# Brown-LEMS/Edge_Based_Visual_Odometry

Hardware: AMD Instinct MI355X
Metric: stereo pairs/sec (TOED+NCC match) on KITTI 1241×376; achieved HBM GB/s (higher is better)
Workload: dtype f64; 1 GPU; configs[1]: single KITTI-shaped stereo pair 1241x376 (generator S2, scene 7+rank, 12 px disparity), TOED both images (fp64, no FMA, bit-exact) + epipolar/disparity/orientation candidate search + NCC, resident in HBM, replayed; toed_mode=hybrid, edges_left=126184, edges_right=126340, candidate_pairs=581657, ncc_matches=472947, sims_stored=False, pairs_in_flight_per_gpu=6, streams_per_gpu=4, pairs_submitted_as_hipgraph=2331, toed_strict_fallbacks=0, parallelism=1 independent sequence(s), one per GPU, no collective

## Files before the change

edge_based_visual_odometry_amd/csrc/ebvo_capi.hip:

```cpp
#include <chrono>
#include <cmath>
#include <cstdio>
#include <cstdlib>
#include <cstring>
#include <new>
#include <utility>

#include "ebvo_internal.h"

const char *const g_kernel_names[K_NUM] = {
    "toed_conv",   "toed_nms",   "toed_rowscan", "toed_compact", "toed_finalize", "toed_exact_centre", "toed_exact_mags", "cand_boxes", "epi_lines",
    "cand_count",  "scan",       "cand_fill",    "edge_patches", "ncc_pairs",     "ncc_stored", "misc", "sobel", "gn_refine", "sift",
    "gt_misc",     "gt_pool",    "gt_census",    "gt_rows",      "tgt_project",   "tgt_veridical", "tgt_rows",
    "pose_cascade"};

int ebvo_fail_hip(ebvo_ctx *ctx, hipError_t e, const char *what, const char *file, int line)
{
    char buf[512];
    snprintf(buf, sizeof buf, "%s failed: %s (%s:%d)", what, hipGetErrorString(e), file, line);
    if (ctx)
        ctx->last_error = buf;
    else
        fprintf(stderr, "[ebvo] %s\n", buf);
    (void)hipGetLastError();
// ... 5090 lines not shown
        EBVO_HIP(ctx, hipMemcpyAsync(base + o_pr, proj_right, sizeof(double) * 2 * nz, hipMemcpyHostToDevice, st));
        if (row_on)
            EBVO_HIP(ctx, hipMemcpyAsync(base + o_on, row_on, nz, hipMemcpyHostToDevice, st));
        else
            EBVO_HIP(ctx, hipMemsetAsync(base + o_on, 1, nz, st));
        EBVO_HIP(ctx, hipMemsetAsync(d_rows, 0, sizeof(int32_t) * 2 * nz, st));
    }
    if ((rc = tgt_rows_enqueue(ctx, s, (const int32_t *)(base + o_rp), (const ebvo_edge *)base, (const ebvo_edge *)(base + o_R), nullptr,
                               nullptr, nullptr, nullptr, (const double *)(base + o_pl), (const double *)(base + o_pr),
                               (const uint8_t *)(base + o_on), n_kf, np, tp_dist, d_rows, (uint8_t *)(base + o_tp), d_tot)))
        return rc;
    std::vector<int32_t> rows(2 * nz + 1);
    unsigned long long tot[5] = {0, 0, 0, 0, 0};
    if (n_kf)
        EBVO_HIP(ctx, hipMemcpyAsync(rows.data(), d_rows, sizeof(int32_t) * 2 * nz, hipMemcpyDeviceToHost, st));
    if (is_tp && np)
        EBVO_HIP(ctx, hipMemcpyAsync(is_tp, base + o_tp, npz, hipMemcpyDeviceToHost, st));
    EBVO_HIP(ctx, hipMemcpyAsync(tot, d_tot, sizeof tot, hipMemcpyDeviceToHost, st));
    EBVO_HIP(ctx, hipStreamSynchronize(st));
    tgt_stage_doubles(rows.data(), row_on, n_kf, stage_out);
    if ((rc = tgt_totals_agree(ctx, *stage_out, tot)))
        return rc;
    if (n_tp && n_kf)
        memcpy(n_tp, rows.data(), sizeof(int32_t) * 2 * nz);
    return EBVO_OK;
}

static bool debug_value_ok(int key, int value)
{
    switch (key)
    {
    case 4: case 7: case 10: case 13: case 14:
        return value <= 1;
    case 8:
        return value == 2 || value == 3;
    case 6:
        return value >= 1;
    case 11: case 12:
        return value <= EBVO_DEBUG_MAX_EXACT_BLOCKS;
    case 9:
        return value <= EBVO_DEBUG_MAX_GN_BLOCKS;
    case 18:
        return value <= 512;
    case 19:
        return value <= EBVO_TOTAL_PARTS;
    case 20:
        return value <= 1 << 20;
    case 21:
        return value <= EBVO_DEBUG_MAX_GT_BLOCKS;
    case 22:
        return value <= EBVO_DEBUG_MAX_TEMPORAL_BLOCKS;
    case EBVO_DEBUG_KEY_FINALIZE_BLOCKS:
        return value <= EBVO_DEBUG_MAX_FINALIZE_BLOCKS;
    case 0: case 1: case 2: case 3: case 5: case 15: case 16: case 17:
        return true;
    default:
        return false;
    }
}

extern "C" int ebvo_debug_set(ebvo_ctx *ctx, int key, int value)
{
    if (!ctx || value < 0 || !debug_value_ok(key, value))
        return EBVO_ERR_ARG;
    ++ctx->graph_gen;
    if (key == 10)
        ctx->use_graphs = value;
    else if (key == 14)
        ctx->no_prep = value;
    else if (key == 11 || key == 12)
        ctx->exact_blocks[key - 11] = value;
    else if (key == 15)
        ctx->repeat_mask = value;
    else if (key == 16)
        ctx->stop_stage = value;
    else if (key == 17)
        ctx->ncc_blocks = value;
    else if (key == 18)
        ctx->small_div = value;
    else if (key == 19)
        ctx->cand_blocks = value;
    else if (key == 20)
        ctx->pose_batch = value;
    else if (key == 21)
        ctx->gt_blocks = value;
    else if (key == 22)
        ctx->temporal_blocks = value;
    else if (key == EBVO_DEBUG_KEY_FINALIZE_BLOCKS)
        ctx->finalize_blocks = value;
    else if (key == 13)
        ctx->ingest_stream = value;
    else if (key == 0)
        ctx->wait_attempts = value;
    else if (key == 1)
        ctx->force_overflow = value;
    else if (key == 2)
        ctx->lanes = value;
    else if (key == 3)
        ctx->prof_only = value - 1;
    else if (key == 4)
        ctx->gn_no_rows = value;
    else if (key == 5)
        ctx->gn_rows_below = value;
    else if (key == 9)
        ctx->gn_persist_blocks = value;
    else if (key == 8)
        ctx->gn_persist_waves = value;
    else if (key == 7)
        ctx->gn_per_iteration_rows = value;
    else
    {
        for (Slot *sl : ctx->slots)
            if (sl->tq_cap > 0 && !sl->tq_in_flight)
                sl->tq_cap = value;
    }
    return EBVO_OK;
}

extern "C" int ebvo_fp64_peak(ebvo_ctx *ctx, int iters, double *tflops_muladd, double *tflops_fma)
{
    if (!ctx || iters <= 0)
        return EBVO_ERR_ARG;
    EBVO_HIP(ctx, hipSetDevice(ctx->device));
    return misc_fp64_peak(ctx, *ctx->slots[0], iters, tflops_muladd, tflops_fma);
}
```

edge_based_visual_odometry_amd/csrc/ebvo_internal.h:

```cpp
#ifndef EBVO_INTERNAL_H
#define EBVO_INTERNAL_H

#include <hip/hip_runtime.h>

#include <cstddef>
#include <cstdint>
#include <string>
#include <vector>

#include "../../include/ebvo_hip.h"

enum KernelId
{
    K_CONV = 0,
    K_NMS,
    K_ROWSCAN,
    K_COMPACT,
    K_FINALIZE,
    K_EXACT_CENTRE,
    K_EXACT_MAGS,
    K_BOXES,
    K_LINES,
    K_CAND_COUNT,
    K_SCAN,
// ... 235 lines not shown
    std::vector<Slot *> slots;
    int kf_n = -1;
    uint64_t kf_gen = 0;
    ebvo_edge *kf_L = nullptr, *kf_R = nullptr;
    float *kf_Ln = nullptr, *kf_Rn = nullptr;
    uint8_t *kf_Lf = nullptr, *kf_Rf = nullptr;
    uint8_t *kf_Ld = nullptr, *kf_Rd = nullptr;
    uint8_t *kf_imgL = nullptr, *kf_imgR = nullptr;
    size_t kf_img_bytes = 0;
    int kf_h = 0, kf_w = 0;
    size_t kf_cap = 0;
    bool undist_on = false;
    ebvo_undistort_params undist{};
    int lanes = 4;
    int prof_only = -1;
    uint64_t submit_seq = 0;
    std::vector<hipStream_t> lane_streams;
    hipStream_t copy_stream = nullptr;
    struct HostRange
    {
        const uint8_t *host = nullptr, *dev = nullptr;
        size_t bytes = 0;
        bool ours = false;
    };
    std::vector<HostRange> host_ranges;
    int64_t pull_uploads = 0, stream_uploads = 0;
    hipStream_t upload_stream = nullptr;
    uint64_t sw_seq = 0;
    uint64_t sw_tag[2] = {0, 0};
    int sw_h = 0, sw_w = 0;
    PinnedBuf sw_toed[2], sw_cand, sw_ncc, sw_up;
    int gn_no_rows = 0;
    int gn_persist_waves = 2;
    int gn_persist_blocks = 0;
    int gn_per_iteration_rows = 0;
    int gn_rows_below = 0;
    int wait_attempts = 0;
    int force_overflow = 0;
    uint64_t graph_gen = 1;
    int use_graphs = 1;
    int64_t graph_launches = 0;
    int exact_blocks[2] = {0, 0};
    int cand_blocks = 0;
    int small_div = 0;
    int ncc_blocks = 0;
    int stop_stage = 0;
    int repeat_mask = 0;
    int no_prep = 0;
    int ingest_stream = 0;
    PoseRng pose_rng;
    int pose_batch = 0;
    int gt_blocks = 0;
    int temporal_blocks = 0;
    int finalize_blocks = 0;
    bool screen_audit = false;
    int64_t toed_fallbacks = 0;

    bool prof = false;
    int prof_every = 1;
    int64_t prof_submits = 0;
    std::vector<ProfEvent> prof_free;
    double prof_ms[K_NUM] = {0};
    int64_t prof_launches[K_NUM] = {0};
};

int ebvo_fail_hip(ebvo_ctx *ctx, hipError_t e, const char *what, const char *file, int line);

struct DevCount
{
    int64_t host;
    const int32_t *dev;
};
#ifdef __HIPCC__
__device__ inline int64_t devcount(const DevCount &c)
{
    if (!c.dev)
        return c.host;
    const int64_t v = *c.dev;
    return v < c.host ? v : c.host;
}
#endif

#define EBVO_HIP(ctx, call)                                              \
    do                                                                   \
    {                                                                    \
        hipError_t e_ = (call);                                          \
        if (e_ != hipSuccess)                                            \
            return ebvo_fail_hip((ctx), e_, #call, __FILE__, __LINE__);  \
    } while (0)

int ebvo_grow(ebvo_ctx *ctx, Slot &s, GrowBuf &b, size_t bytes);

bool ebvo_prof_begin(ebvo_ctx *ctx, Slot &s, int kid);
void ebvo_prof_end(ebvo_ctx *ctx, Slot &s);

bool ebvo_prof_kernel(ebvo_ctx *ctx, Slot &s, int kid, hipEvent_t *a, hipEvent_t *b);

struct ProfScope
{
    ebvo_ctx *c;
    Slot &s;
    bool on;
    ProfScope(ebvo_ctx *ctx, Slot &slot, int kid) : c(ctx), s(slot), on(ebvo_prof_begin(ctx, slot, kid)) {}
    ~ProfScope()
    {
        if (on)
// ... 192 lines not shown
```

edge_based_visual_odometry_amd/csrc/toed_kernels.hip:

```cpp
#include <cstring>

#include <hip/hip_ext.h>

#include "ebvo_internal.h"
#include <atomic>
#include "ebvo_math.h"

namespace
{

const double h_TAP_INT[4][19] = {
    {7.99187055345274e-06, 6.69151128824427e-05, 0.000436341347522880, 0.00221592420596900,
     0.00876415024678427, 0.0269954832565940, 0.0647587978329459, 0.120985362259572, 0.176032663382150,
     0.199471140200716, 0.176032663382150, 0.120985362259572, 0.0647587978329459, 0.0269954832565940,
     0.00876415024678427, 0.00221592420596900, 0.000436341347522880, 6.69151128824427e-05,
     7.99187055345274e-06},
    {1.79817087452687e-05, 0.000133830225764885, 0.000763597358165040, 0.00332388630895351,
     0.0109551878084803, 0.0269954832565940, 0.0485690983747094, 0.0604926811297858, 0.0440081658455374, 0,
     -0.0440081658455374, -0.0604926811297858, -0.0485690983747094, -0.0269954832565940,
     -0.0109551878084803, -0.00332388630895351, -0.000763597358165040, -0.000133830225764885,
     -1.79817087452687e-05},
    {3.84608770384913e-05, 0.000250931673309160, 0.00122721003990810, 0.00443184841193801,
     0.0115029471989044, 0.0202466124424455, 0.0202371243227956, 0, -0.0330061243841531,
     -0.0498677850501791, -0.0330061243841531, 0, 0.0202371243227956, 0.0202466124424455,
// ... 1003 lines not shown
                f[7] += cc[3] * rr[0];
                f[8] += cc[0] * rr[3];
            }
            else
            {
                EBVO_ACCUM9(f, cc, rr)
            }
        }
    }
}

template <int SY, int SX>
__device__ inline double exact_mag(const uint8_t *__restrict__ img, int h, int w, const ExactTaps &L, int I, int J)
{
    constexpr bool IP = (SY == 0 && SX == 0);
    const int i = I >> 1, j = J >> 1;
    const double(*ck)[4] = L.tap[SX];
    const double(*rk)[4] = L.tap[SY];
    double fx = 0.0, fy = 0.0;
    constexpr int PM = IP ? 8 : 9;
    const bool fast = __all(window_inside(h, w, i, j));
    const ColMask cm = column_mask(w, j);
    Row24 nxt = fetch_row(img, h, w, i + PM, j);
#pragma unroll 1
    for (int p = -PM; p <= PM; ++p)
    {
        const Row24 cur = nxt;
        nxt = fetch_row(img, h, w, i - min(p + 1, PM), j);
        int vb[19];
        unpack_row(cur, h, i - p, cm, fast, vb);
        const double r0 = rk[p + 9][0], r1 = rk[p + 9][1];
        int lz = 0;
        asm volatile("" : "+v"(lz));
        const double(*ckl)[4] = ck + lz;
#pragma unroll
        for (int q = -PM; q <= PM; ++q)
        {
            const double v = (double)vb[q + 9];
            if (IP)
            {
                fx += v * L.prod[p + 8][q + 8][0];
                fy += v * L.prod[p + 8][q + 8][1];
            }
            else
            {
                fx += (v * ckl[q + 9][1]) * r0;
                fy += (v * ckl[q + 9][0]) * r1;
            }
        }
    }
    return sqrt(fx * fx + fy * fy);
}

#ifdef EBVO_WAVE_TRACE
__device__ unsigned long long g_wave_trace[2][8192 * 4];
__device__ inline void wave_trace(int which, int wave, unsigned long long t0, int tasks)
{
    if ((threadIdx.x & 63) == 0 && wave < 8192)
    {
        const unsigned hw = __builtin_amdgcn_s_getreg(4 | (0 << 6) | (31 << 11));
        const unsigned xcc = __builtin_amdgcn_s_getreg(20 | (0 << 6) | (31 << 11));
        unsigned long long *o = g_wave_trace[which] + (size_t)wave * 4;
        o[0] = t0;
        o[1] = __builtin_amdgcn_s_memrealtime();
        o[2] = ((unsigned long long)xcc << 32) | hw;
        o[3] = (unsigned long long)tasks;
    }
}
extern "C" int ebvo_wave_trace_read(int which, unsigned long long *dst, int n_waves)
{
    return (int)hipMemcpyFromSymbol(dst, HIP_SYMBOL(g_wave_trace), (size_t)n_waves * 32, (size_t)which * 8192 * 32,
                                    hipMemcpyDeviceToHost);
}
#define EBVO_TRACE_BEGIN() const unsigned long long trace_t0 = __builtin_amdgcn_s_memrealtime(); int trace_n = 0
#define EBVO_TRACE_TASK() ++trace_n
#define EBVO_TRACE_END(which) wave_trace(which, wave, trace_t0, trace_n)
#else
#define EBVO_TRACE_BEGIN()
#define EBVO_TRACE_TASK()
#define EBVO_TRACE_END(which)
#endif

struct ExactTask
{
    int im, ph, k0, n;
};

__device__ inline bool exact_task(const ExactBatch &E, int n_img, int cap, int list0, int t, ExactTask &o)
{
    int base = 0;
    for (int ph = 0; ph < 4; ++ph)
        for (int im = 0; im < n_img; ++im)
        {
            const int n = min(E.lcount[im][list0 + ph], cap);
            const int c = (n + 63) >> 6;
            if (t < base + c)
            {
                o.im = im;
                o.ph = ph;
                o.k0 = (t - base) << 6;
                o.n = n;
                return true;
            }
            base += c;
        }
    return false;
}

template <int SY, int SX>
__device__ inline void centre_run(const ExactBatch &E, const ExactTaps &L, int h, int w, int cap, int im, int k, int n)
{
    const int W2 = 2 * w, H2 = 2 * h, wpr = (W2 + 31) >> 5;
    constexpr int PH = (SY << 1) | SX;
    const int32_t *__restrict__ list = E.lists[im] + (size_t)PH * cap;
    CandExact *__restrict__ cd = E.cd[im];
    const uint8_t *__restrict__ flag = E.flag[im];
    if (k < n)
    {
        const int t = list[k];
        const int o = E.src[im][2 * t];
        const int I = o / W2, J = o - I * W2;
        double f[9];
        exact9<SY, SX>(E.img[im], h, w, L, I >> 1, J >> 1, f);
        const double gx = f[0], gy = f[1];
        const double m = sqrt(gx * gx + gy * gy);
        NmsSector S;
        int packed = -1;
        if (nms_sector(m, gx, gy, S))
        {
            packed = (S.a1 + 1) | ((S.b1 + 1) << 2) | ((S.a2 + 1) << 4) | ((S.b2 + 1) << 6);
#pragma unroll
            for (int q = 0; q < 4; ++q)
            {
                const int da = (q & 2) ? S.a2 : S.a1, db = (q & 2) ? S.b2 : S.b1;
                const int nI = (q & 1) ? I - da : I + da, nJ = (q & 1) ? J - db : J + db;
                const int no = nI * W2 + nJ;
                const bool is_cand = nI >= 10 && nI < H2 - 10 && nJ >= 10 && nJ < W2 - 10 && flag[no] == 1;
                if (!is_cand)
                    atomicOr(&E.needbits[im][(size_t)nI * wpr + (nJ >> 5)], 1u << (nJ & 31));
            }
        }
        CandExact r;
        r.gx = gx;
        r.gy = gy;
        r.m = m;
        third_order_dir(f, r.tox, r.toy);
        r.sector = packed;
        r.pad0 = 0;
        r.pad1[0] = r.pad1[1] = 0.0;
        cd[t] = r;
        E.magmap[im][mag_index(I, J, W2)] = m;
    }
}

#ifndef EBVO_CENTRE_WPS
#define EBVO_CENTRE_WPS 0
#endif
#if EBVO_CENTRE_WPS > 0
__global__ __launch_bounds__(256, EBVO_CENTRE_WPS) void toed_exact_centre_kernel(ExactBatch E, const ToedTables *__restrict__ T, int h,
#else
__global__ __launch_bounds__(256) void toed_exact_centre_kernel(ExactBatch E, const ToedTables *__restrict__ T, int h,
#endif
                                                                int w, int cap, int n_img)
{
    __shared__ ExactTaps L;
    EBVO_TRACE_BEGIN();
    load_exact_taps(L, T);
    const int lane = threadIdx.x & 63;
    const int wave = __builtin_amdgcn_readfirstlane((int)(blockIdx.x * 4 + (threadIdx.x >> 6)));
    ExactTask q;
    for (int t = wave; exact_task(E, n_img, cap, 0, t, q); t += gridDim.x * 4)
    {
        EBVO_TRACE_TASK();
        switch (q.ph)
        {
        case 0: centre_run<0, 0>(E, L, h, w, cap, q.im, q.k0 + lane, q.n); break;
        case 1: centre_run<0, 1>(E, L, h, w, cap, q.im, q.k0 + lane, q.n); break;
        case 2: centre_run<1, 0>(E, L, h, w, cap, q.im, q.k0 + lane, q.n); break;
        default: centre_run<1, 1>(E, L, h, w, cap, q.im, q.k0 + lane, q.n); break;
        }
    }
    EBVO_TRACE_END(0);
}

__global__ __launch_bounds__(256) void toed_need_count_kernel(ExactBatch E, int h, int w)
{
    const int W2 = 2 * w, H2 = 2 * h, wpr = (W2 + 31) >> 5;
    const int im = blockIdx.y, I = blockIdx.x * 4 + (threadIdx.x >> 6), lane = threadIdx.x & 63;
    if (I >= H2)
        return;
    const uint32_t *__restrict__ row = E.needbits[im] + (size_t)I * wpr;
    int ne = 0, no = 0;
    for (int k = lane; k < wpr; k += 64)
    {
        const uint32_t v = row[k];
        ne += __popc(v & 0x55555555u);
        no += __popc(v & 0xaaaaaaaau);
    }
    for (int d = 32; d > 0; d >>= 1)
    {
        ne += __shfl_down(ne, d);
        no += __shfl_down(no, d);
    }
    if (lane == 0)
    {
        E.need_cnt[im][I] = ne;
        E.need_cnt[im][H2 + I] = no;
    }
}

__global__ __launch_bounds__(256) void toed_need_compact_kernel(ExactBatch E, int h, int w, int cap)
{
    const int W2 = 2 * w, H2 = 2 * h, wpr = (W2 + 31) >> 5;
    const int I = blockIdx.x, im = blockIdx.y;
    const int32_t *__restrict__ cnt = E.need_cnt[im];
    const bool last = I >= H2 - 2;
    const int mine0 = cnt[I], mine1 = cnt[H2 + I];
    if (!last && mine0 + mine1 == 0)
        return;
    const uint32_t *__restrict__ bits = E.needbits[im];
    int32_t *__restrict__ lists = E.lists[im];
    __shared__ int w_par[2][4], s_sum[4][2];
    const int lane = threadIdx.x & 63, wid = threadIdx.x >> 6;
    int a0 = 0, a1 = 0;
    for (int r = (I & 1) + 2 * threadIdx.x; r < I; r += 512)
    {
        a0 += cnt[r];
        a1 += cnt[H2 + r];
    }
    for (int d = 32; d > 0; d >>= 1)
    {
        a0 += __shfl_down(a0, d);
        a1 += __shfl_down(a1, d);
    }
    if (lane == 0)
    {
        s_sum[wid][0] = a0;
        s_sum[wid][1] = a1;
    }
    __syncthreads();
    int base_ph[2] = {s_sum[0][0] + s_sum[1][0] + s_sum[2][0] + s_sum[3][0], s_sum[0][1] + s_sum[1][1] + s_sum[2][1] + s_sum[3][1]};
    if (last && threadIdx.x == 0)
    {
        const int n0 = base_ph[0] + mine0, n1 = base_ph[1] + mine1;
        E.lcount[im][4 + 2 * (I & 1) + 0] = n0;
        E.lcount[im][4 + 2 * (I & 1) + 1] = n1;
        atomicAdd(const_cast<int32_t *>(E.counts[im]) + 3, n0 + n1);
    }
    if (mine0 + mine1 == 0)
        return;
    const int par = threadIdx.x & 1;
    const unsigned long long pmask = par ? 0xaaaaaaaaaaaaaaaaull : 0x5555555555555555ull;
    for (int J0 = 0; J0 < W2; J0 += 256)
    {
        const int J = J0 + threadIdx.x;
        const int o = I * W2 + J;
        const bool f = J < W2 && ((bits[(size_t)I * wpr + (J >> 5)] >> (J & 31)) & 1u);
        const unsigned long long m_all = __ballot(f);
        const unsigned long long below = (1ull << lane) - 1ull;
        if (lane == 0)
        {
            w_par[0][wid] = __popcll(m_all & 0x5555555555555555ull);
            w_par[1][wid] = __popcll(m_all & 0xaaaaaaaaaaaaaaaaull);
        }
        __syncthreads();
        int pre_ph = 0, tot_ph[2] = {0, 0};
#pragma unroll
        for (int k = 0; k < 4; ++k)
        {
            if (k < wid)
                pre_ph += w_par[par][k];
            tot_ph[0] += w_par[0][k];
            tot_ph[1] += w_par[1][k];
        }
        if (f)
        {
            const int ph = ((I & 1) << 1) | par;
            const int pos = base_ph[par] + pre_ph + __popcll(m_all & pmask & below);
            if (pos < cap)
                lists[(size_t)(4 + ph) * cap + pos] = o;
        }
        base_ph[0] += tot_ph[0];
        base_ph[1] += tot_ph[1];
        __syncthreads();
    }
}

template <int SY, int SX>
__device__ inline void mags_run(const ExactBatch &E, const ExactTaps &L, int h, int w, int cap, int im, int k, int n)
{
    const int W2 = 2 * w;
    constexpr int PH = (SY << 1) | SX;
    const int32_t *__restrict__ list = E.lists[im] + (size_t)(4 + PH) * cap;
    if (k < n)
    {
        const int o = list[k];
        const int I = o / W2, J = o - I * W2;
        E.magmap[im][mag_index(I, J, W2)] = exact_mag<SY, SX>(E.img[im], h, w, L, I, J);
    }
}

__global__ __launch_bounds__(256) void toed_exact_mags_kernel(ExactBatch E, const ToedTables *__restrict__ T, int h,
                                                              int w, int cap, int n_img)
{
    __shared__ ExactTaps L;
    EBVO_TRACE_BEGIN();
    load_exact_taps(L, T);
    const int lane = threadIdx.x & 63;
    const int wave = __builtin_amdgcn_readfirstlane((int)(blockIdx.x * 4 + (threadIdx.x >> 6)));
    ExactTask q;
    for (int t = wave; exact_task(E, n_img, cap, 4, t, q); t += gridDim.x * 4)
    {
        EBVO_TRACE_TASK();
        switch (q.ph)
        {
        case 0: mags_run<0, 0>(E, L, h, w, cap, q.im, q.k0 + lane, q.n); break;
        case 1: mags_run<0, 1>(E, L, h, w, cap, q.im, q.k0 + lane, q.n); break;
        case 2: mags_run<1, 0>(E, L, h, w, cap, q.im, q.k0 + lane, q.n); break;
        default: mags_run<1, 1>(E, L, h, w, cap, q.im, q.k0 + lane, q.n); break;
        }
    }
    EBVO_TRACE_END(1);
}

__global__ __launch_bounds__(256) void toed_exact_decide_kernel(ExactBatch E, int h, int w, int cap)
{
    __shared__ int s_cnt[4][2];
    const int im = blockIdx.y, W2 = 2 * w;
    const CandExact *__restrict__ cd = E.cd[im];
    CandRec *__restrict__ rec = E.rec[im];
    int32_t *__restrict__ ft = E.cand_flag[im], *__restrict__ fk = ft + cap;
    const int n = min(E.counts[im][2], cap);
    for (int c = blockIdx.x; c * 256 < n; c += gridDim.x)
    {
        const int t = c * 256 + threadIdx.x;
        bool is_max = false;
        int kept = 0;
        if (t < n)
        {
            const int o = E.src[im][2 * t];
            const int I = o / W2, J = o - I * W2;
            const CandExact ce = cd[t];
            const double gx = ce.gx, gy = ce.gy, m = ce.m;
            NmsSector S;
            double px = 0, py = 0, sm = 0;
            if (ce.sector >= 0 && nms_sector(m, gx, gy, S))
            {
                const double *__restrict__ mm = E.magmap[im];
                is_max = nms_finish(m, S, I, J, mm[mag_index(I + S.a1, J + S.b1, W2)], mm[mag_index(I + S.a2, J + S.b2, W2)],
                                    mm[mag_index(I - S.a1, J - S.b1, W2)], mm[mag_index(I - S.a2, J - S.b2, W2)], px, py, sm);
            }
            CandRec r;
            r.x = r.y = r.smag = 0.0;
            r.tox = ce.tox;
            r.toy = ce.toy;
            if (is_max)
            {
                r.x = (px - 1) / 2;
                r.y = (py - 1) / 2;
                r.smag = sm;
                kept = (r.x > 10 && r.x < w - 10 && r.y > 10 && r.y < h - 10) ? 1 : 0;
            }
            rec[t] = r;
            ft[t] = is_max ? 1 : 0;
            fk[t] = kept;
        }
        const unsigned long long bm = __ballot(is_max), bk = __ballot(kept != 0);
        if ((threadIdx.x & 63) == 0)
        {
            s_cnt[threadIdx.x >> 6][0] = __popcll(bm);
            s_cnt[threadIdx.x >> 6][1] = __popcll(bk);
        }
        __syncthreads();
        if (threadIdx.x == 0)
            E.chunk_cnt[im][c] = make_int2(s_cnt[0][0] + s_cnt[1][0] + s_cnt[2][0] + s_cnt[3][0],
                                           s_cnt[0][1] + s_cnt[1][1] + s_cnt[2][1] + s_cnt[3][1]);
        __syncthreads();
    }
}


__global__ __launch_bounds__(256) void toed_screen_audit_kernel(ExactBatch E, ScreenDiag D, int h, int w, int cap, int im,
                                                                unsigned long long *out)
{
    const int W2 = 2 * w, H2 = 2 * h;
    const size_t plane = (size_t)H2 * W2;
    const float *__restrict__ dp = D.plane[im];
    const int n = min(E.counts[im][2], cap);
    double e[4] = {0, 0, 0, 0};
    for (int t = blockIdx.x * blockDim.x + threadIdx.x; t < n; t += gridDim.x * blockDim.x)
    {
        const int o = E.src[im][2 * t];
        const CandExact ce = E.cd[im][t];
        e[0] = fmax(e[0], fabs((double)dp[o] - ce.gx));
        e[1] = fmax(e[1], fabs((double)dp[plane + o] - ce.gy));
        e[2] = fmax(e[2], fabs((double)dp[2 * plane + o] - ce.m));
    }
    for (int ph = 0; ph < 4; ++ph)
    {
        const int32_t *__restrict__ list = E.lists[im] + (size_t)(4 + ph) * cap;
        const int np = min(E.lcount[im][4 + ph], cap);
        for (int k = blockIdx.x * blockDim.x + threadIdx.x; k < np; k += gridDim.x * blockDim.x)
        {
            const int o = list[k];
            const int I = o / W2, J = o - I * W2;
            if (I >= 10 && I < H2 - 10 && J >= 10 && J < W2 - 10)
                e[3] = fmax(e[3], fabs((double)dp[2 * plane + o] - E.magmap[im][mag_index(I, J, W2)]));
        }
    }
#pragma unroll
    for (int k = 0; k < 4; ++k)
        if (e[k] > 0)
            atomicMax(&out[k], (unsigned long long)__double_as_longlong(e[k]));
    if (blockIdx.x == 0 && threadIdx.x == 0)
        out[5] = (unsigned long long)n;
}

__global__ __launch_bounds__(256) void toed_cand_scatter_kernel(ImgBatch B, int cap)
{
    __shared__ int s_base[4][2], s_in[4][2];
    const CandRec *__restrict__ rec = B.rec[blockIdx.y];
    const int32_t *__restrict__ ftp = B.cand_flag[blockIdx.y], *__restrict__ fkp = ftp + cap;
    const int2 *__restrict__ chunk_cnt = reinterpret_cast<const int2 *>(B.cand_off[blockIdx.y]);
    ebvo_edge *__restrict__ edges = B.edges[blockIdx.y];
    double *__restrict__ all4 = B.all4[blockIdx.y];
    int32_t *counts = B.counts[blockIdx.y];
    const int n = min(counts[2], cap);
    const int lane = threadIdx.x & 63, wid = threadIdx.x >> 6;
    if (n == 0 && blockIdx.x == 0 && threadIdx.x == 0)
    {
        counts[0] = 0;
        counts[1] = 0;
    }
    for (int c = blockIdx.x; c * 256 < n; c += gridDim.x)
    {
        int a0 = 0, a1 = 0;
        for (int k = threadIdx.x; k < c; k += 256)
        {
            const int2 v = chunk_cnt[k];
            a0 += v.x;
            a1 += v.y;
        }
        for (int d = 32; d > 0; d >>= 1)
        {
            a0 += __shfl_down(a0, d);
            a1 += __shfl_down(a1, d);
        }
        const int t = c * 256 + threadIdx.x;
        const int f_t = t < n ? ftp[t] : 0, f_k = t < n ? fkp[t] : 0;
        const unsigned long long bm = __ballot(f_t != 0), bk = __ballot(f_k != 0);
        if (lane == 0)
        {
            s_base[wid][0] = a0;
            s_base[wid][1] = a1;
            s_in[wid][0] = __popcll(bm);
            s_in[wid][1] = __popcll(bk);
        }
        __syncthreads();
        int o_t = s_base[0][0] + s_base[1][0] + s_base[2][0] + s_base[3][0];
        int o_k = s_base[0][1] + s_base[1][1] + s_base[2][1] + s_base[3][1];
// ... 182 lines not shown
                    D.plane[k] = (float *)((int32_t *)(s.im[k].maps + mag_map_doubles(H2, W2)) + need_words + 4 * H2);
                hipLaunchKernelGGL(toed_screen_fused_kernel<true>, ftiles, dim3(256), 0, s.stream, B,
                                   (const ToedTables *)g_tables_dev[ctx->device], h, w, D);
            }
            else
                hipLaunchKernelGGL(toed_screen_fused_kernel<false>, ftiles, dim3(256), 0, s.stream, B,
                                   (const ToedTables *)g_tables_dev[ctx->device], h, w, D);
        }
        const int stop = ctx->stop_stage;
        if (stop == 1)
            return EBVO_OK;
        {
            ProfScope ps(ctx, s, K_COMPACT);
            hipLaunchKernelGGL(toed_compact_phase_kernel, dim3(H2 - 20, n_img), dim3(256), 0, s.stream, B, h, w, cap);
        }
        if (stop == 2)
            return EBVO_OK;
        {
            ExactBatch E{};
            for (int k = 0; k < n_img; ++k)
            {
                ImageWS &ws = s.im[k];
                E.img[k] = ws.img;
                E.src[k] = ws.src;
                E.counts[k] = ws.counts;
                E.lists[k] = ws.cand_lists;
                E.lcount[k] = ws.cand_lcount;
                E.cd[k] = (CandExact *)ws.cand_data;
                E.rec[k] = (CandRec *)ws.cand_rec;
                E.cand_flag[k] = ws.cand_flag;
                E.chunk_cnt[k] = reinterpret_cast<int2 *>(ws.cand_off);
                E.flag[k] = ws.flag;
                E.magmap[k] = ws.maps;
                E.needbits[k] = (uint32_t *)(ws.maps + mag_map_doubles(H2, W2));
                E.need_cnt[k] = (int32_t *)(E.needbits[k] + need_words);
            }
            const ToedTables *T = (const ToedTables *)g_tables_dev[ctx->device];
            {
                hipEvent_t k_begin, k_end;
                if (ebvo_prof_kernel(ctx, s, K_EXACT_CENTRE, &k_begin, &k_end))
                    hipExtLaunchKernelGGL(toed_exact_centre_kernel, dim3(resident_blocks(ctx, 0)), dim3(256), 0, s.stream,
                                          k_begin, k_end, 0, E, T, h, w, cap, n_img);
                else
                    hipLaunchKernelGGL(toed_exact_centre_kernel, dim3(resident_blocks(ctx, 0)), dim3(256), 0, s.stream, E,
                                       T, h, w, cap, n_img);
                if (ctx->repeat_mask & 1)
                    hipLaunchKernelGGL(toed_exact_centre_kernel, dim3(resident_blocks(ctx, 0)), dim3(256), 0, s.stream, E,
                                       T, h, w, cap, n_img);
            }
            if (stop == 3)
                return EBVO_OK;
            {
                ProfScope ps(ctx, s, K_COMPACT);
                hipLaunchKernelGGL(toed_need_count_kernel, dim3((H2 + 3) / 4, n_img), dim3(256), 0, s.stream, E, h, w);
                hipLaunchKernelGGL(toed_need_compact_kernel, dim3(H2, n_img), dim3(256), 0, s.stream, E, h, w, cap);
            }
            if (stop == 4)
                return EBVO_OK;
            {
                ProfScope ps(ctx, s, K_EXACT_MAGS);
                hipLaunchKernelGGL(toed_exact_mags_kernel, dim3(resident_blocks(ctx, 1)), dim3(256), 0, s.stream, E, T, h,
                                   w, cap, n_img);
                if (ctx->repeat_mask & 2)
                    hipLaunchKernelGGL(toed_exact_mags_kernel, dim3(resident_blocks(ctx, 1)), dim3(256), 0, s.stream, E, T, h,
                                       w, cap, n_img);
                if (stop == 5)
                    return EBVO_OK;
                hipLaunchKernelGGL(toed_exact_decide_kernel, dim3(512 / (ctx->small_div > 0 ? ctx->small_div : 4), n_img), dim3(256), 0, s.stream, E, h, w, cap);
            }
            if (stop == 6)
                return EBVO_OK;
            if (ctx->screen_audit)
                for (int k = 0; k < n_img; ++k)
                {
                    unsigned long long *out = toed_screen_audit_result(s, k, h, w);
                    EBVO_HIP(ctx, hipMemsetAsync(out, 0, 8 * sizeof(unsigned long long), s.stream));
                    hipLaunchKernelGGL(toed_screen_audit_kernel, dim3(512), dim3(256), 0, s.stream, E, D, h, w, cap, k, out);
                }
        }
        if (ev_conv_end)
            EBVO_HIP(ctx, hipEventRecord(ev_conv_end, s.stream));
        {
            ProfScope ps(ctx, s, K_FINALIZE);
            hipLaunchKernelGGL(toed_cand_scatter_kernel, dim3(512 / (ctx->small_div > 0 ? ctx->small_div : 4), n_img), dim3(256), 0, s.stream, B, cap);
        }
        if (ev_end)
            EBVO_HIP(ctx, hipEventRecord(ev_end, s.stream));
        EBVO_HIP(ctx, hipGetLastError());
        return EBVO_OK;
    }
    if (ev_conv_begin)
        EBVO_HIP(ctx, hipEventRecord(ev_conv_begin, s.stream));
    {
        ProfScope ps(ctx, s, K_CONV);
        dim3 grid((w + TILE_W - 1) / TILE_W, (h + TILE_H - 1) / TILE_H, 2 * n_img);
        hipLaunchKernelGGL(toed_conv_kernel, grid, dim3(256), 0, s.stream, B,
                           (const ToedTables *)g_tables_dev[ctx->device], h, w);
    }
    if (ev_conv_end)
        EBVO_HIP(ctx, hipEventRecord(ev_conv_end, s.stream));
    {
        ProfScope ps(ctx, s, K_NMS);
        dim3 grid((W2 - 20 + 63) / 64, (H2 - 20 + 3) / 4, n_img);
        hipLaunchKernelGGL(toed_nms_kernel, grid, dim3(64, 4), 0, s.stream, B, h, w);
    }
    {
        ProfScope ps(ctx, s, K_ROWSCAN);
        hipLaunchKernelGGL(toed_rowscan_kernel, dim3(n_img), dim3(64), 0, s.stream, B, H2, 0);
// ... 15 lines not shown
```

Before: 3506 stereo pairs/s.

## Pair vertically adjacent exact-magnitude points to share image row fetches

Rewrites the need-list count and compact kernels to work on 4-row bands. Within a band they classify needed sub-pixel points into singles and vertically close pairs in the same column, encoding the row distance in the high bits of each list entry. The exact-magnitude kernel gains pair and mixed integer/half-row paths that compute two magnitudes from one pass over the 19-20 image rows, so row loads and tap products are shared. The change adds more list classes, extra shared tap tables and a launch-bounds occupancy hint, plus a debug key that restores single-point processing.

```diff
diff --git a/edge_based_visual_odometry_amd/csrc/ebvo_capi.hip b/edge_based_visual_odometry_amd/csrc/ebvo_capi.hip
--- a/edge_based_visual_odometry_amd/csrc/ebvo_capi.hip
+++ b/edge_based_visual_odometry_amd/csrc/ebvo_capi.hip
@@ -5166,6 +5166,8 @@
         return value <= EBVO_DEBUG_MAX_TEMPORAL_BLOCKS;
     case EBVO_DEBUG_KEY_FINALIZE_BLOCKS:
         return value <= EBVO_DEBUG_MAX_FINALIZE_BLOCKS;
+    case 25:
+        return value <= 1;
     case 0: case 1: case 2: case 3: case 5: case 15: case 16: case 17:
         return true;
     default:
@@ -5202,6 +5204,8 @@
         ctx->temporal_blocks = value;
     else if (key == EBVO_DEBUG_KEY_FINALIZE_BLOCKS)
         ctx->finalize_blocks = value;
+    else if (key == 25)
+        ctx->mags_singles = value;
     else if (key == 13)
         ctx->ingest_stream = value;
     else if (key == 0)
diff --git a/edge_based_visual_odometry_amd/csrc/ebvo_internal.h b/edge_based_visual_odometry_amd/csrc/ebvo_internal.h
--- a/edge_based_visual_odometry_amd/csrc/ebvo_internal.h
+++ b/edge_based_visual_odometry_amd/csrc/ebvo_internal.h
@@ -311,6 +311,7 @@
     int pose_batch = 0;
     int gt_blocks = 0;
     int temporal_blocks = 0;
+    int mags_singles = 0;
     int finalize_blocks = 0;
     bool screen_audit = false;
     int64_t toed_fallbacks = 0;
diff --git a/edge_based_visual_odometry_amd/csrc/toed_kernels.hip b/edge_based_visual_odometry_amd/csrc/toed_kernels.hip
--- a/edge_based_visual_odometry_amd/csrc/toed_kernels.hip
+++ b/edge_based_visual_odometry_amd/csrc/toed_kernels.hip
@@ -1079,6 +1079,106 @@
     return sqrt(fx * fx + fy * fy);
 }
 
+struct PairTaps
+{
+    double rz[2][21][2];
+    double zrow[17][2];
+};
+
+__device__ inline void load_pair_taps(PairTaps &P, const ToedTables *__restrict__ T)
+{
+    for (int t = threadIdx.x; t < 2 * 21 * 2; t += blockDim.x)
+    {
+        const int half = t / 42, k = (t % 42) / 2, d = t & 1;
+        P.rz[half][k][d] = (k == 0 || k == 20) ? 0.0 : (half ? T->tap_half[d][k - 1] : T->tap_int[d][k - 1]);
+    }
+    for (int t = threadIdx.x; t < 17 * 2; t += blockDim.x)
+        P.zrow[t >> 1][t & 1] = 0.0;
+    __syncthreads();
+}
+
+template <int SX>
+__device__ inline void exact_mag_pair(const uint8_t *__restrict__ img, int h, int w, const ExactTaps &L, const PairTaps &P,
+                                      int IA, int IB, int J, double &mA, double &mB)
+{
+    const int iA = IA >> 1, iB = IB >> 1, j = J >> 1;
+    const int top = iB + 9;
+    const double(*ck)[4] = L.tap[SX];
+    const double(*rzA)[2] = P.rz[IA & 1] + (1 - (iB - iA));
+    const double(*rzB)[2] = P.rz[IB & 1] + 1;
+    const int n = __any(iB != iA) ? 20 : 19;
+    double fxA = 0.0, fyA = 0.0, fxB = 0.0, fyB = 0.0;
+    const bool fast = __all(window_inside(h, w, iA, j) && window_inside(h, w, iB, j));
+    const ColMask cm = column_mask(w, j);
+    Row24 nxt = fetch_row(img, h, w, top, j);
+#pragma unroll 1
+    for (int s = 0; s < n; ++s)
+    {
+        const Row24 cur = nxt;
+        nxt = fetch_row(img, h, w, top - min(s + 1, n - 1), j);
+        int vb[19];
+        unpack_row(cur, h, top - s, cm, fast, vb);
+        const double a0 = rzA[s][0], a1 = rzA[s][1], b0 = rzB[s][0], b1 = rzB[s][1];
+        int lz = 0;
+        asm volatile("" : "+v"(lz));
+        const double(*ckl)[4] = ck + lz;
+#pragma unroll
+        for (int q = -9; q <= 9; ++q)
+        {
+            const double v = (double)vb[q + 9];
+            const double cx = v * ckl[q + 9][1], cy = v * ckl[q + 9][0];
+            fxA += cx * a0;
+            fyA += cy * a1;
+            fxB += cx * b0;
+            fyB += cy * b1;
+        }
+    }
+    mA = sqrt(fxA * fxA + fyA * fyA);
+    mB = sqrt(fxB * fxB + fyB * fyB);
+}
+
+__device__ inline void exact_mag_mixed(const uint8_t *__restrict__ img, int h, int w, const ExactTaps &L, const PairTaps &P,
+                                       int IN, int IG, int J, double &mN, double &mG)
+{
+    const int iN = IN >> 1, iG = IG >> 1, j = J >> 1;
+    const int top = iG + 9;
+    const double(*ck)[4] = L.tap[0];
+    const double(*rk)[4] = L.tap[1];
+    const int shift = iN - iG - 1;
+    double fxN = 0.0, fyN = 0.0, fxG = 0.0, fyG = 0.0;
+    const bool fast = __all(window_inside(h, w, iN, j) && window_inside(h, w, iG, j));
+    const ColMask cm = column_mask(w, j);
+    Row24 nxt = fetch_row(img, h, w, top, j);
+#pragma unroll 1
+    for (int s = 0; s < 19; ++s)
+    {
+        const Row24 cur = nxt;
+        nxt = fetch_row(img, h, w, top - min(s + 1, 18), j);
+        int vb[19];
+        unpack_row(cur, h, top - s, cm, fast, vb);
+        const double r0 = rk[s][0], r1 = rk[s][1];
+        const int pn = s + shift;
+        const double(*pr)[2] = (pn >= 0 && pn <= 16) ? L.prod[pn] : P.zrow;
+        int lz = 0;
+        asm volatile("" : "+v"(lz));
+        const double(*ckl)[4] = ck + lz;
+#pragma unroll
+        for (int q = -9; q <= 9; ++q)
+        {
+            const double v = (double)vb[q + 9];
+            if (q >= -8 && q <= 8)
+            {
+                fxN += v * pr[q + 8][0];
+                fyN += v * pr[q + 8][1];
+            }
+            fxG += (v * ckl[q + 9][1]) * r0;
+            fyG += (v * ckl[q + 9][0]) * r1;
+        }
+    }
+    mN = sqrt(fxN * fxN + fyN * fyN);
+    mG = sqrt(fxG * fxG + fyG * fyG);
+}
+
 #ifdef EBVO_WAVE_TRACE
 __device__ unsigned long long g_wave_trace[2][8192 * 4];
 __device__ inline void wave_trace(int which, int wave, unsigned long long t0, int tasks)
@@ -1113,24 +1213,31 @@
     int im, ph, k0, n;
 };
 
-__device__ inline bool exact_task(const ExactBatch &E, int n_img, int cap, int list0, int t, ExactTask &o)
+constexpr int MAGS_N_LISTS = 7;
+__device__ constexpr int MAGS_LIST_ORDER[MAGS_N_LISTS] = {8, 9, 10, 7, 5, 6, 4};
+
+template <bool MAGS>
+__device__ inline bool exact_task(const ExactBatch &E, int n_img, int cap, int t, ExactTask &o)
 {
     int base = 0;
-    for (int ph = 0; ph < 4; ++ph)
+    for (int ph = 0; ph < (MAGS ? MAGS_N_LISTS : 4); ++ph)
+    {
+        const int li = MAGS ? MAGS_LIST_ORDER[ph] : ph;
         for (int im = 0; im < n_img; ++im)
         {
-            const int n = min(E.lcount[im][list0 + ph], cap);
+            const int n = min(E.lcount[im][li], cap);
             const int c = (n + 63) >> 6;
             if (t < base + c)
             {
                 o.im = im;
-                o.ph = ph;
+                o.ph = li;
                 o.k0 = (t - base) << 6;
                 o.n = n;
                 return true;
             }
             base += c;
         }
+    }
     return false;
 }
 
@@ -1196,7 +1303,7 @@
     const int lane = threadIdx.x & 63;
     const int wave = __builtin_amdgcn_readfirstlane((int)(blockIdx.x * 4 + (threadIdx.x >> 6)));
     ExactTask q;
-    for (int t = wave; exact_task(E, n_img, cap, 0, t, q); t += gridDim.x * 4)
+    for (int t = wave; exact_task<false>(E, n_img, cap, t, q); t += gridDim.x * 4)
     {
         EBVO_TRACE_TASK();
         switch (q.ph)
@@ -1210,106 +1317,248 @@
     EBVO_TRACE_END(0);
 }
 
-__global__ __launch_bounds__(256) void toed_need_count_kernel(ExactBatch E, int h, int w)
-{
-    const int W2 = 2 * w, H2 = 2 * h, wpr = (W2 + 31) >> 5;
-    const int im = blockIdx.y, I = blockIdx.x * 4 + (threadIdx.x >> 6), lane = threadIdx.x & 63;
-    if (I >= H2)
+constexpr int NEED_BAND = 4;
+__host__ __device__ constexpr unsigned need_rule(unsigned bits, int col_parity, bool pairs)
+{
+    unsigned code = 0;
+    int pending = -1;
+    for (int r = 0; r < NEED_BAND; ++r)
+    {
+        if (!((bits >> r) & 1u))
+            continue;
+        if (pending < 0 || !pairs)
+        {
+            if (pending >= 0)
+                code |= 1u << (4 * pending);
+            pending = r;
+        }
+        else if (col_parity == 0 && (pending & 1) == 0 && (r & 1) == 0)
+        {
+            code |= 1u << (4 * pending);
+            pending = r;
+        }
+        else
+        {
+            code |= (unsigned)(4 + (r - pending)) << (4 * pending);
+            pending = -1;
+        }
+    }
+    if (pending >= 0)
+        code |= 1u << (4 * pending);
+    return code;
+}
+
+struct BandMasks
+{
+    uint32_t s[4], p01, p02, p03, p12, p13, p23;
+};
+__host__ __device__ constexpr BandMasks band_masks(uint32_t a, uint32_t b, uint32_t c, uint32_t d, bool pairs)
+{
+    BandMasks m{};
+    if (!pairs)
+    {
+        m.s[0] = a, m.s[1] = b, m.s[2] = c, m.s[3] = d;
+        return m;
+    }
+    constexpr uint32_t EVEN = 0x55555555u;
+    m.p01 = a & b;
+    uint32_t q0 = a & ~b, q1 = b & ~a, q2 = 0;
+    m.s[0] = q0 & c & EVEN;
+    m.p02 = q0 & c & ~EVEN;
+    m.p12 = q1 & c;
+    q2 = c & ~(m.p02 | m.p12);
+    q0 &= ~c;
+    q1 &= ~c;
+    m.p03 = q0 & d;
+    m.p13 = q1 & d;
+    m.p23 = q2 & d;
+    m.s[0] |= q0 & ~d;
+    m.s[1] = q1 & ~d;
+    m.s[2] = q2 & ~d;
+    m.s[3] = d & ~(q0 | q1 | q2);
+    return m;
+}
+__host__ __device__ constexpr bool band_masks_follow_rule()
+{
+    for (int pairs = 0; pairs < 2; ++pairs)
+        for (unsigned bits = 0; bits < 16; ++bits)
+            for (int par = 0; par < 2; ++par)
+            {
+                const auto w = [&](int r) { return ((bits >> r) & 1u) << par; };
+                const BandMasks m = band_masks(w(0), w(1), w(2), w(3), pairs != 0);
+                const auto g = [&](uint32_t v) { return (v >> par) & 1u; };
+                unsigned code = 0;
+                for (int r = 0; r < 4; ++r)
+                    code |= g(m.s[r]) << (4 * r);
+                code |= g(m.p01) * 5u | g(m.p02) * 6u | g(m.p03) * 7u;
+                code |= (g(m.p12) * 5u | g(m.p13) * 6u) << 4;
+                code |= (g(m.p23) * 5u) << 8;
+                if (code != need_rule(bits, par, pairs != 0))
+                    return false;
+            }
+    return true;
+}
+static_assert(NEED_BAND == 4 && band_masks_follow_rule(), "band_masks must be need_rule on 32 columns");
+
+constexpr int NEED_CLASSES = 7;
+constexpr int NEED_PAIR_SHIFT = 29;
+struct BandClasses
+{
+    uint32_t m[NEED_CLASSES][6];
+};
+constexpr int NEED_SRC_N[NEED_CLASSES] = {2, 2, 2, 2, 6, 1, 4};
+constexpr int NEED_SRC_ROW[NEED_CLASSES][6] = {{0, 2}, {0, 2}, {1, 3}, {1, 3}, {0, 0, 0, 1, 1, 2}, {1}, {0, 0, 1, 2}};
+constexpr int NEED_SRC_DIST[NEED_CLASSES][6] = {{0, 0}, {0, 0}, {0, 0}, {0, 0}, {1, 2, 3, 1, 2, 1}, {2}, {1, 3, 1, 1}};
+__device__ inline BandClasses band_classes(uint32_t a, uint32_t b, uint32_t c, uint32_t d, bool pairs)
+{
+    constexpr uint32_t EVEN = 0x55555555u, ODD = 0xaaaaaaaau;
+    const BandMasks k = band_masks(a, b, c, d, pairs);
+    BandClasses o{};
+    o.m[0][0] = k.s[0] & EVEN, o.m[0][1] = k.s[2] & EVEN;
+    o.m[1][0] = k.s[0] & ODD, o.m[1][1] = k.s[2] & ODD;
+    o.m[2][0] = k.s[1] & EVEN, o.m[2][1] = k.s[3] & EVEN;
+    o.m[3][0] = k.s[1] & ODD, o.m[3][1] = k.s[3] & ODD;
+    o.m[4][0] = k.p01 & ODD, o.m[4][1] = k.p02 & ODD, o.m[4][2] = k.p03 & ODD;
+    o.m[4][3] = k.p12 & ODD, o.m[4][4] = k.p13 & ODD, o.m[4][5] = k.p23 & ODD;
+    o.m[5][0] = k.p13 & EVEN;
+    o.m[6][0] = k.p01 & EVEN, o.m[6][1] = k.p03 & EVEN, o.m[6][2] = k.p12 & EVEN, o.m[6][3] = k.p23 & EVEN;
+    return o;
+}
+
+__device__ inline void band_words(const uint32_t *__restrict__ bits, int H2, int wpr, int band, int k, uint32_t v[4])
+{
+#pragma unroll
+    for (int r = 0; r < NEED_BAND; ++r)
+    {
+        const int I = band * NEED_BAND + r;
+        v[r] = I < H2 ? bits[(size_t)I * wpr + k] : 0u;
+    }
+}
+
+__device__ inline int wave_sum(int v)
+{
+    for (int d = 32; d > 0; d >>= 1)
+        v += __shfl_xor(v, d);
+    return v;
+}
+
+__global__ __launch_bounds__(256) void toed_need_count_kernel(ExactBatch E, int h, int w, int pairs)
+{
+    const int W2 = 2 * w, H2 = 2 * h, wpr = (W2 + 31) >> 5, nb = (H2 + NEED_BAND - 1) / NEED_BAND;
+    const int im = blockIdx.y, band = blockIdx.x * 4 + (threadIdx.x >> 6), lane = threadIdx.x & 63;
+    if (band >= nb)
         return;
-    const uint32_t *__restrict__ row = E.needbits[im] + (size_t)I * wpr;
-    int ne = 0, no = 0;
+    int n[NEED_CLASSES] = {0, 0, 0, 0, 0, 0, 0};
     for (int k = lane; k < wpr; k += 64)
     {
-        const uint32_t v = row[k];
-        ne += __popc(v & 0x55555555u);
-        no += __popc(v & 0xaaaaaaaau);
-    }
-    for (int d = 32; d > 0; d >>= 1)
-    {
-        ne += __shfl_down(ne, d);
-        no += __shfl_down(no, d);
-    }
-    if (lane == 0)
-    {
-        E.need_cnt[im][I] = ne;
-        E.need_cnt[im][H2 + I] = no;
-    }
-}
-
-__global__ __launch_bounds__(256) void toed_need_compact_kernel(ExactBatch E, int h, int w, int cap)
-{
-    const int W2 = 2 * w, H2 = 2 * h, wpr = (W2 + 31) >> 5;
-    const int I = blockIdx.x, im = blockIdx.y;
+        uint32_t v[4];
+        band_words(E.needbits[im], H2, wpr, band, k, v);
+        if ((v[0] | v[1] | v[2] | v[3]) == 0u)
+            continue;
+        const BandClasses bc = band_classes(v[0], v[1], v[2], v[3], pairs != 0);
+#pragma unroll
+        for (int c = 0; c < NEED_CLASSES; ++c)
+#pragma unroll
+            for (int q = 0; q < NEED_SRC_N[c]; ++q)
+                n[c] += __popc(bc.m[c][q]);
+    }
+#pragma unroll
+    for (int c = 0; c < NEED_CLASSES; ++c)
+    {
+        const int t = wave_sum(n[c]);
+        if (lane == 0)
+            E.need_cnt[im][c * nb + band] = t;
+    }
+}
+
+constexpr int NEED_WAVE_OF[NEED_CLASSES] = {2, 2, 3, 3, 0, 1, 1};
+__global__ __launch_bounds__(256) void toed_need_compact_kernel(ExactBatch E, int h, int w, int cap, int pairs)
+{
+    const int W2 = 2 * w, H2 = 2 * h, wpr = (W2 + 31) >> 5, nb = (H2 + NEED_BAND - 1) / NEED_BAND;
+    const int im = blockIdx.y, band = blockIdx.x, lane = threadIdx.x & 63;
+    const int wid = __builtin_amdgcn_readfirstlane((int)(threadIdx.x >> 6));
     const int32_t *__restrict__ cnt = E.need_cnt[im];
-    const bool last = I >= H2 - 2;
-    const int mine0 = cnt[I], mine1 = cnt[H2 + I];
-    if (!last && mine0 + mine1 == 0)
+    const bool publish = band == nb - 1 && wid == 0;
+    int mine = 0;
+#pragma unroll
+    for (int c = 0; c < NEED_CLASSES; ++c)
+        if (NEED_WAVE_OF[c] == wid)
+            mine += cnt[c * nb + band];
+    if (!publish && mine == 0)
         return;
-    const uint32_t *__restrict__ bits = E.needbits[im];
+    int base[NEED_CLASSES];
+#pragma unroll
+    for (int c = 0; c < NEED_CLASSES; ++c)
+    {
+        base[c] = 0;
+        if (NEED_WAVE_OF[c] == wid || publish)
+        {
+            int a = 0;
+            for (int r = lane; r < band; r += 64)
+                a += cnt[c * nb + r];
+            base[c] = wave_sum(a);
+        }
+    }
+    if (publish && lane == 0)
+    {
+        int points = 0;
+#pragma unroll
+        for (int c = 0; c < NEED_CLASSES; ++c)
+        {
+            const int n = base[c] + cnt[c * nb + band];
+            E.lcount[im][4 + c] = n;
+            points += c < 4 ? n : 2 * n;
+        }
+        atomicAdd(const_cast<int32_t *>(E.counts[im]) + 3, points);
+    }
+    if (mine == 0)
+        return;
     int32_t *__restrict__ lists = E.lists[im];
-    __shared__ int w_par[2][4], s_sum[4][2];
-    const int lane = threadIdx.x & 63, wid = threadIdx.x >> 6;
-    int a0 = 0, a1 = 0;
-    for (int r = (I & 1) + 2 * threadIdx.x; r < I; r += 512)
-    {
-        a0 += cnt[r];
-        a1 += cnt[H2 + r];
-    }
-    for (int d = 32; d > 0; d >>= 1)
-    {
-        a0 += __shfl_down(a0, d);
-        a1 += __shfl_down(a1, d);
-    }
-    if (lane == 0)
-    {
-        s_sum[wid][0] = a0;
-        s_sum[wid][1] = a1;
-    }
-    __syncthreads();
-    int base_ph[2] = {s_sum[0][0] + s_sum[1][0] + s_sum[2][0] + s_sum[3][0], s_sum[0][1] + s_sum[1][1] + s_sum[2][1] + s_sum[3][1]};
-    if (last && threadIdx.x == 0)
-    {
-        const int n0 = base_ph[0] + mine0, n1 = base_ph[1] + mine1;
-        E.lcount[im][4 + 2 * (I & 1) + 0] = n0;
-        E.lcount[im][4 + 2 * (I & 1) + 1] = n1;
-        atomicAdd(const_cast<int32_t *>(E.counts[im]) + 3, n0 + n1);
-    }
-    if (mine0 + mine1 == 0)
-        return;
-    const int par = threadIdx.x & 1;
-    const unsigned long long pmask = par ? 0xaaaaaaaaaaaaaaaaull : 0x5555555555555555ull;
-    for (int J0 = 0; J0 < W2; J0 += 256)
-    {
-        const int J = J0 + threadIdx.x;
-        const int o = I * W2 + J;
-        const bool f = J < W2 && ((bits[(size_t)I * wpr + (J >> 5)] >> (J & 31)) & 1u);
-        const unsigned long long m_all = __ballot(f);
-        const unsigned long long below = (1ull << lane) - 1ull;
-        if (lane == 0)
-        {
-            w_par[0][wid] = __popcll(m_all & 0x5555555555555555ull);
-            w_par[1][wid] = __popcll(m_all & 0xaaaaaaaaaaaaaaaaull);
-        }
-        __syncthreads();
-        int pre_ph = 0, tot_ph[2] = {0, 0};
-#pragma unroll
-        for (int k = 0; k < 4; ++k)
-        {
-            if (k < wid)
-                pre_ph += w_par[par][k];
-            tot_ph[0] += w_par[0][k];
-            tot_ph[1] += w_par[1][k];
-        }
-        if (f)
-        {
-            const int ph = ((I & 1) << 1) | par;
-            const int pos = base_ph[par] + pre_ph + __popcll(m_all & pmask & below);
-            if (pos < cap)
-                lists[(size_t)(4 + ph) * cap + pos] = o;
-        }
-        base_ph[0] += tot_ph[0];
-        base_ph[1] += tot_ph[1];
-        __syncthreads();
+    for (int k0 = 0; k0 < wpr; k0 += 64)
+    {
+        const int k = k0 + lane;
+        uint32_t v[4] = {0u, 0u, 0u, 0u};
+        if (k < wpr)
+            band_words(E.needbits[im], H2, wpr, band, k, v);
+        const BandClasses bc = band_classes(v[0], v[1], v[2], v[3], pairs != 0);
+#pragma unroll
+        for (int c = 0; c < NEED_CLASSES; ++c)
+        {
+            if (NEED_WAVE_OF[c] != wid)
+                continue;
+            int n = 0;
+#pragma unroll
+            for (int q = 0; q < NEED_SRC_N[c]; ++q)
+                n += __popc(bc.m[c][q]);
+            int incl = n;
+            for (int d = 1; d < 64; d <<= 1)
+            {
+                const int up = __shfl_up(incl, d);
+                if (lane >= d)
+                    incl += up;
+            }
+            const int lane_base = base[c] + incl - n;
+            base[c] += __shfl(incl, 63);
+            int32_t *__restrict__ list = lists + (size_t)(4 + c) * cap;
+#pragma unroll
+            for (int q = 0; q < NEED_SRC_N[c]; ++q)
+            {
+                uint32_t mq = bc.m[c][q];
+                while (mq)
+                {
+                    const int j = __ffs(mq) - 1;
+                    mq &= mq - 1u;
+                    const uint32_t below = (1u << j) - 1u;
+                    int pos = lane_base;
+#pragma unroll
+                    for (int q2 = 0; q2 < NEED_SRC_N[c]; ++q2)
+                        pos += __popc(bc.m[c][q2] & below) + (q2 < q ? (int)((bc.m[c][q2] >> j) & 1u) : 0);
+                    if (pos < cap)
+                        list[pos] = ((band * NEED_BAND + NEED_SRC_ROW[c][q]) * W2 + (k << 5) + j) |
+                                    (NEED_SRC_DIST[c][q] << NEED_PAIR_SHIFT);
+                }
+            }
+        }
     }
 }
 
@@ -1327,24 +1576,56 @@
     }
 }
 
-__global__ __launch_bounds__(256) void toed_exact_mags_kernel(ExactBatch E, const ToedTables *__restrict__ T, int h,
+template <int C>
+__device__ inline void mags_pair_run(const ExactBatch &E, const ExactTaps &L, const PairTaps &P, int h, int w, int cap, int im,
+                                     int k, int n)
+{
+    const int W2 = 2 * w;
+    const int32_t *__restrict__ list = E.lists[im] + (size_t)(4 + C) * cap;
+    if (k < n)
+    {
+        const int e = list[k];
+        const int o = e & ((1 << NEED_PAIR_SHIFT) - 1);
+        const int IA = o / W2, J = o - IA * W2, IB = IA + (e >> NEED_PAIR_SHIFT);
+        double mA, mB;
+        if (C == 6)
+        {
+            const bool a_int = (IA & 1) == 0;
+            double mN, mG;
+            exact_mag_mixed(E.img[im], h, w, L, P, a_int ? IA : IB, a_int ? IB : IA, J, mN, mG);
+            mA = a_int ? mN : mG;
+            mB = a_int ? mG : mN;
+        }
+        else
+            exact_mag_pair<C == 4 ? 1 : 0>(E.img[im], h, w, L, P, IA, IB, J, mA, mB);
+        E.magmap[im][mag_index(IA, J, W2)] = mA;
+        E.magmap[im][mag_index(IB, J, W2)] = mB;
+    }
+}
+
+__global__ __launch_bounds__(256, 6) void toed_exact_mags_kernel(ExactBatch E, const ToedTables *__restrict__ T, int h,
                                                               int w, int cap, int n_img)
 {
     __shared__ ExactTaps L;
+    __shared__ PairTaps P;
     EBVO_TRACE_BEGIN();
+    load_pair_taps(P, T);
     load_exact_taps(L, T);
     const int lane = threadIdx.x & 63;
     const int wave = __builtin_amdgcn_readfirstlane((int)(blockIdx.x * 4 + (threadIdx.x >> 6)));
     ExactTask q;
-    for (int t = wave; exact_task(E, n_img, cap, 4, t, q); t += gridDim.x * 4)
+    for (int t = wave; exact_task<true>(E, n_img, cap, t, q); t += gridDim.x * 4)
     {
         EBVO_TRACE_TASK();
         switch (q.ph)
         {
-        case 0: mags_run<0, 0>(E, L, h, w, cap, q.im, q.k0 + lane, q.n); break;
-        case 1: mags_run<0, 1>(E, L, h, w, cap, q.im, q.k0 + lane, q.n); break;
-        case 2: mags_run<1, 0>(E, L, h, w, cap, q.im, q.k0 + lane, q.n); break;
-        default: mags_run<1, 1>(E, L, h, w, cap, q.im, q.k0 + lane, q.n); break;
+        case 4: mags_run<0, 0>(E, L, h, w, cap, q.im, q.k0 + lane, q.n); break;
+        case 5: mags_run<0, 1>(E, L, h, w, cap, q.im, q.k0 + lane, q.n); break;
+        case 6: mags_run<1, 0>(E, L, h, w, cap, q.im, q.k0 + lane, q.n); break;
+        case 7: mags_run<1, 1>(E, L, h, w, cap, q.im, q.k0 + lane, q.n); break;
+        case 8: mags_pair_run<4>(E, L, P, h, w, cap, q.im, q.k0 + lane, q.n); break;
+        case 9: mags_pair_run<5>(E, L, P, h, w, cap, q.im, q.k0 + lane, q.n); break;
+        default: mags_pair_run<6>(E, L, P, h, w, cap, q.im, q.k0 + lane, q.n); break;
         }
     }
     EBVO_TRACE_END(1);
@@ -1423,16 +1704,21 @@
         e[1] = fmax(e[1], fabs((double)dp[plane + o] - ce.gy));
         e[2] = fmax(e[2], fabs((double)dp[2 * plane + o] - ce.m));
     }
-    for (int ph = 0; ph < 4; ++ph)
-    {
-        const int32_t *__restrict__ list = E.lists[im] + (size_t)(4 + ph) * cap;
-        const int np = min(E.lcount[im][4 + ph], cap);
+    for (int c = 0; c < NEED_CLASSES; ++c)
+    {
+        const int32_t *__restrict__ list = E.lists[im] + (size_t)(4 + c) * cap;
+        const int np = min(E.lcount[im][4 + c], cap);
         for (int k = blockIdx.x * blockDim.x + threadIdx.x; k < np; k += gridDim.x * blockDim.x)
         {
-            const int o = list[k];
-            const int I = o / W2, J = o - I * W2;
-            if (I >= 10 && I < H2 - 10 && J >= 10 && J < W2 - 10)
-                e[3] = fmax(e[3], fabs((double)dp[2 * plane + o] - E.magmap[im][mag_index(I, J, W2)]));
+            const int en = list[k];
+            const int oA = en & ((1 << NEED_PAIR_SHIFT) - 1), dist = en >> NEED_PAIR_SHIFT;
+            for (int pt = 0; pt < (dist ? 2 : 1); ++pt)
+            {
+                const int o = oA + pt * dist * W2;
+                const int I = o / W2, J = o - I * W2;
+                if (I >= 10 && I < H2 - 10 && J >= 10 && J < W2 - 10)
+                    e[3] = fmax(e[3], fabs((double)dp[2 * plane + o] - E.magmap[im][mag_index(I, J, W2)]));
+            }
         }
     }
 #pragma unroll
@@ -1721,8 +2007,10 @@
                 return EBVO_OK;
             {
                 ProfScope ps(ctx, s, K_COMPACT);
-                hipLaunchKernelGGL(toed_need_count_kernel, dim3((H2 + 3) / 4, n_img), dim3(256), 0, s.stream, E, h, w);
-                hipLaunchKernelGGL(toed_need_compact_kernel, dim3(H2, n_img), dim3(256), 0, s.stream, E, h, w, cap);
+                const int pairs = !ctx->mags_singles && (long long)H2 * W2 < (1ll << NEED_PAIR_SHIFT);
+                const int bands = (H2 + NEED_BAND - 1) / NEED_BAND;
+                hipLaunchKernelGGL(toed_need_count_kernel, dim3((bands + 3) / 4, n_img), dim3(256), 0, s.stream, E, h, w, pairs);
+                hipLaunchKernelGGL(toed_need_compact_kernel, dim3(bands, n_img), dim3(256), 0, s.stream, E, h, w, cap, pairs);
             }
             if (stop == 4)
                 return EBVO_OK;
```

Result: no change. 3539 stereo pairs/s (median of 6 runs) (+0.9%).
